# rasoolims/ImageTranslate

Hardware: AMD Instinct MI355X
Metric: train tokens/sec (whole node), 6L enc-dec d=512 seq128 b64, 1/2/4/8 GPU (higher is better)
Workload: dtype bf16; 1 GPU; 6L/6L enc-dec d=512 h=8 ff=2048 V=30000, src[64,128] tgt[64,128], synthetic random-token MT; global_batch=64, seq_len=128, parallelism=dp1, distinct_batches=8, directions=2

## Files before the change

imagetranslate_amd/_lib.py:

```python
import ctypes
import os
from ctypes import POINTER, Structure, c_char_p, c_float, c_int, c_int32, c_int64, c_uint64, c_void_p

_HERE = os.path.dirname(os.path.abspath(__file__))
LIB_PATH = os.environ.get("IMT_LIB") or os.path.join(_HERE, "libimt_hip.so")

IMT_F32, IMT_BF16 = 0, 1
IMT_NT, IMT_NN, IMT_TN = 0, 1, 2
IMT_AUX_NONE, IMT_AUX_GELU_FWD, IMT_AUX_DGELU, IMT_AUX_SPLITK_WS = 0, 1, 2, 3


class GemmArgs(Structure):
    _fields_ = [
        ("dtype", c_int32), ("layout", c_int32),
        ("M", c_int32), ("N", c_int32), ("K", c_int32),
        ("A", c_void_p), ("lda", c_int64),
        ("B", c_void_p), ("ldb", c_int64),
        ("C", c_void_p), ("ldc", c_int64),
        ("c_dtype", c_int32), ("accumulate", c_int32),
        ("bias", c_void_p),
        ("resid", c_void_p), ("ldr", c_int64),
        ("aux", c_void_p), ("ldaux", c_int64),
        ("aux_mode", c_int32), ("split_k", c_int32),
        ("alpha", c_float), ("dropout_p", c_float),
# ... 126 lines not shown
        ("x", c_void_p), ("ldx", c_int64),
        ("w", c_void_p), ("ldw", c_int64),
        ("bias", c_void_p), ("target", c_void_p),
        ("logprob", c_void_p), ("lse", c_void_p),
        ("seg_offsets", c_void_p), ("n_seg", c_int32), ("normalize", c_int32),
        ("seg_score", c_void_p),
        ("ws", c_void_p), ("ws_bytes", c_int64),
    ]


_P = c_void_p
SIGNATURES = {
    "imt_version": (c_int, []),
    "imt_last_error": (c_char_p, []),
    "imt_gemm": (c_int, [POINTER(GemmArgs), _P]),
    "imt_gemm_grouped_tn": (c_int, [POINTER(GemmArgs), c_int, _P]),
    "imt_gemm_splitk_ws_bytes": (c_int64, []),
    "imt_gemm_bias_residual_ln_supported": (c_int, [c_int, c_int, c_int]),
    "imt_gemm_bias_residual_ln": (c_int, [c_int, _P, c_int64, _P, c_int64, _P, _P, c_int64, _P, _P, _P, _P, c_int64, _P, _P, c_int, c_int,
                                          c_int, c_float, c_float, c_uint64, _P]),
    "imt_colsum": (c_int, [c_int, _P, c_int64, c_int, c_int, _P, _P, _P]),
    "imt_layernorm_fwd": (c_int, [c_int, _P, _P, _P, _P, _P, _P, c_int, c_int, c_float, c_float, c_uint64, _P]),
    "imt_add_layernorm_fwd": (c_int, [c_int, _P, _P, _P, _P, _P, _P, _P, _P, c_int, c_int, c_float, c_float, c_uint64, _P]),
    "imt_embed_ln_fwd": (c_int, [c_int, _P, _P, _P, _P, _P, _P, _P, _P, _P, _P, _P, _P, c_int, c_int, c_int, c_int, c_int, c_int, c_float,
                                 c_float, c_uint64, _P]),
    "imt_layernorm_bwd": (c_int, [c_int, _P, _P, _P, _P, _P, _P, _P, _P, c_int, c_int, c_float, c_uint64, _P, c_float,
                                  c_uint64, _P, _P]),
    "imt_embed_fwd": (c_int, [c_int, _P, _P, _P, _P, _P, _P, _P, c_int, c_int, c_int, c_int, c_int, c_int, _P]),
    "imt_embed_bwd": (c_int, [c_int, _P, _P, _P, _P, _P, _P, _P, c_int, c_int, c_int, c_int64, _P]),
    "imt_attention_fwd": (c_int, [POINTER(AttnArgs), _P]),
    "imt_attention_bwd": (c_int, [POINTER(AttnArgs), _P]),
    "imt_attention_qkv_fwd_supported": (c_int, [c_int, c_int, c_int, c_int, c_int, c_int, c_int]),
    "imt_attention_qkv_fwd": (c_int, [POINTER(AttnArgs), _P, c_int64, _P, _P, c_int, _P]),
    "imt_gather_rows": (c_int, [c_int, _P, c_int64, _P, _P, c_int64, c_int, c_int, _P]),
    "imt_scatter_rows": (c_int, [c_int, _P, c_int64, _P, _P, c_int64, c_int, c_int, _P]),
    "imt_log_softmax_fwd": (c_int, [c_int, _P, c_int64, _P, c_int64, _P, c_int, c_int, _P]),
    "imt_log_softmax_bwd": (c_int, [_P, c_int64, _P, c_int64, c_int, _P, c_int64, c_int, c_int, _P]),
    "imt_smoothed_nll_fwd": (c_int, [_P, c_int64, _P, _P, c_int, c_int, c_float, c_int64, _P]),
    "imt_smoothed_nll_bwd": (c_int, [_P, _P, _P, c_int64, c_int, c_int, c_float, c_int64, _P]),
    "imt_xent_fused_fwd_bwd": (c_int, [c_int, _P, c_int64, _P, _P, c_int, c_int, c_float, c_int64, c_float, _P]),
    "imt_score_ws_bytes": (c_int64, [c_int, c_int]),
    "imt_score_supported": (c_int, [c_int, c_int, c_int]),
    "imt_score_rows": (c_int, [POINTER(ScoreArgs), _P]),
    "imt_scaled_sum": (c_int, [_P, c_int, c_float, _P, _P]),
    "imt_sumsq": (c_int, [_P, c_int64, _P, _P, _P]),
    "imt_ln_partial_reduce": (c_int, [_P, c_int, c_int, _P, _P, _P, _P]),
    "imt_clip_adam": (c_int, [_P, _P, _P, _P, _P, c_int64, _P, c_float, c_float, c_float, c_float, c_float, c_float,
                              c_int64, c_int, _P]),
    "imt_clip_scale": (c_int, [_P, c_int64, _P, c_float, c_float, _P]),
    "imt_cast_f32_to_bf16": (c_int, [_P, _P, c_int64, _P]),
    "imt_gated_mix": (c_int, [c_int, _P, _P, _P, _P, c_int64, c_int, _P]),
    "imt_add_rows_dropout": (c_int, [c_int, _P, c_int, _P, _P, c_int64, c_int, c_int, c_float, c_uint64, _P]),
    "imt_obj_rows": (c_int, [c_int, c_int, _P, _P, _P, _P, _P, _P, _P, c_int64, c_int, c_int, _P, _P]),
    "imt_relu_dropout": (c_int, [c_int, _P, c_int64, c_int, c_float, c_uint64, _P]),
    "imt_relu_dropout_bwd": (c_int, [c_int, _P, _P, _P, c_int64, c_int, c_float, c_uint64, _P]),
    "imt_obj_fold_w": (c_int, [_P, _P, c_int, c_int, _P]),
    "imt_obj_embed_grad": (c_int, [c_int, _P, _P, c_int64, _P, c_int64, c_int, _P]),
    "imt_gated_mix_bwd": (c_int, [c_int, _P, _P, _P, _P, _P, _P, _P, _P, c_int64, c_int, _P]),
    "imt_attn_pool_plan": (c_int, [c_int, c_int, c_int]),
    "imt_attn_pool_fwd": (c_int, [c_int, _P, _P, _P, _P, _P, _P, _P, c_int64, c_int, c_int, _P]),
    "imt_attn_pool_bwd": (c_int, [c_int, _P, _P, _P, _P, _P, _P, _P, _P, _P, _P, _P, _P, c_int64, c_int, c_int, _P]),
    "imt_contrastive": (c_int, [_P, _P, _P, _P, _P, _P, c_int, c_int, c_int, _P]),
    "imt_sent_pool_fwd": (c_int, [c_int, _P, _P, _P, _P, _P, _P, c_int64, c_int, c_int, c_float, c_uint64, _P]),
    "imt_sent_pool_bwd": (c_int, [c_int, _P, _P, _P, _P, _P, _P, _P, _P, _P, c_int64, c_int, c_int, c_float, c_uint64, _P]),
    "imt_l2_dist": (c_int, [c_int, _P, _P, _P, _P, _P, c_int, c_int64, _P]),
    "imt_comm_unique_id_bytes": (c_int, []),
# ... 66 lines not shown
```

imagetranslate_amd/csrc/attention.hip:

```cpp
#include <stdlib.h>
#include "mma.hpp"

namespace {

struct AttnP {
  int B, H, Tq, Tk;
  const void* Q; int64_t ldq;
  const void* K; int64_t ldk;
  const void* V; int64_t ldv;
  void* O; int64_t ldo;
  float* lse;
  const uint8_t* key_mask;
  const uint8_t* query_mask;
  const uint8_t* mask3d;
  int causal;
  float scale;
  uint32_t drop_thresh; float inv_keep; uint64_t seed;
  const void* dO; int64_t lddo;
  void* dQ; int64_t lddq;
  void* dK; int64_t lddk;
  void* dV; int64_t lddv;
  unsigned long long* trace;
  float* delta;
};
// ... 455 lines not shown
        float pv = (i < p.Tq && j < p.Tk) ? __expf(v - lse_t[il]) : 0.f;
        float dpv = dp[mt][e], pdv = pv;
        if (p.drop_thresh) {
          const bool keep = attn_drop_keep(attn_drop_word(dropout_key(p.seed), attn_pair_row(p, b, h, i) + (uint64_t)(j >> 1)), j, p.drop_thresh);
          dpv = keep ? dpv * p.inv_keep : 0.f;
          pdv = keep ? pv * p.inv_keep : 0.f;
        }
        pd[mt][e] = pdv;
        s[mt][e] = pv * (dpv - delta_t[il]);
      }
#pragma unroll
    for (int u = 0; u < AccOperand<T>::NFR; ++u) {
      const frag_t pf = AccOperand<T>::get(pd, u);
      const frag_t dsf = AccOperand<T>::get(s, u);
#pragma unroll
      for (int dt = 0; dt < NDT; ++dt) {
        mma16(dv[dt], AccOperand<T>::template lds<RB>(dOt, u, 16 * dt), pf);
        mma16(dk[dt], AccOperand<T>::template lds<RB>(Qt, u, 16 * dt), dsf);
      }
    }
    }
  }
  if (j < p.Tk) {
    T* dKb = reinterpret_cast<T*>(p.dK) + ((int64_t)b * p.Tk + j) * p.lddk + h * DH;
    T* dVb = reinterpret_cast<T*>(p.dV) + ((int64_t)b * p.Tk + j) * p.lddv + h * DH;
#pragma unroll
    for (int dt = 0; dt < NDT; ++dt) {
      Vec4<T>::store(dKb + 16 * dt + 4 * g, dk[dt] * p.scale);
      Vec4<T>::store(dVb + 16 * dt + 4 * g, dv[dt]);
    }
  }
}

template <int DH, bool MASK3D>
__global__ __launch_bounds__(512, 4) void attn_bwd_fused_kernel(AttnP p) {
  typedef bf16_t T;
  constexpr int RB = DH * 2, NS = RB / 64, NDT = DH / 16;
  typedef typename Frag<T>::type frag_t;
  extern __shared__ __attribute__((aligned(16))) char smem[];
  char* Qs = smem;
  char* dOs = Qs + 128 * RB;
  char* dST = dOs + 128 * RB;
  float* lse_s = reinterpret_cast<float*>(dST + 128 * 256);
  float* delta_s = lse_s + 128;
  uint8_t* qmask_s = reinterpret_cast<uint8_t*>(delta_s + 128);

  const int lid = imt_xcd_block(blockIdx.x, gridDim.x);
  const int b = lid / p.H, h = lid % p.H;
  const int wave = threadIdx.x >> 6, lane = threadIdx.x & 63, r = lane & 15, g = lane >> 4;
  const T* Qb = reinterpret_cast<const T*>(p.Q) + (int64_t)b * p.Tq * p.ldq + h * DH;
  const T* Kb = reinterpret_cast<const T*>(p.K) + (int64_t)b * p.Tk * p.ldk + h * DH;
  const T* Vb = reinterpret_cast<const T*>(p.V) + (int64_t)b * p.Tk * p.ldv + h * DH;
  const T* dOb = reinterpret_cast<const T*>(p.dO) + (int64_t)b * p.Tq * p.lddo + h * DH;
  const T* Ob = reinterpret_cast<const T*>(p.O) + (int64_t)b * p.Tq * p.ldo + h * DH;

  IMT_STAMP(p.trace, 0);
  const int k0 = 16 * wave;
  const int j = k0 + r;
  frag_t kf[NS], vf[NS];
  bool key_ok;
  {
    constexpr int CPR = RB / 16, NIT = 128 * CPR / 512;
    u32x4 vq[NIT], vo[NIT];
#pragma unroll
    for (int it = 0; it < NIT; ++it) {
      const int q = threadIdx.x + it * 512, tr = min(q / CPR, p.Tq - 1), c = q % CPR;
      vq[it] = *reinterpret_cast<const u32x4*>(Qb + (int64_t)tr * p.ldq + c * 8);
      vo[it] = *reinterpret_cast<const u32x4*>(dOb + (int64_t)tr * p.lddo + c * 8);
    }
    const int i = 16 * wave + r;
    frag_t of[NS], dof[NS];
    load_row_frags<T, DH>(of, Ob, p.ldo, 16 * wave, p.Tq);
    load_row_frags<T, DH>(dof, dOb, p.lddo, 16 * wave, p.Tq);
    load_row_frags<T, DH>(kf, Kb, p.ldk, k0, p.Tk);
    load_row_frags<T, DH>(vf, Vb, p.ldv, k0, p.Tk);
    const float lse_v = p.lse[((int64_t)b * p.H + h) * p.Tq + min(i, p.Tq - 1)];
    const uint8_t* qmp = p.query_mask ? p.query_mask + (int64_t)b * p.Tq + min(i, p.Tq - 1) : reinterpret_cast<const uint8_t*>(Qb);
    const uint8_t* kmp = p.key_mask ? p.key_mask + (int64_t)b * p.Tk + min(j, p.Tk - 1) : reinterpret_cast<const uint8_t*>(Kb);
    const uint8_t qmv = *qmp, kmv = *kmp;
#pragma unroll
    for (int it = 0; it < NIT; ++it) {
      const int q = threadIdx.x + it * 512, tr = q / CPR, c = q % CPR;
      const u32x4 z = {0u, 0u, 0u, 0u};
      *reinterpret_cast<u32x4*>(Qs + tile_off<RB>(tr, c)) = (tr < p.Tq) ? vq[it] : z;
      *reinterpret_cast<u32x4*>(dOs + tile_off<RB>(tr, c)) = (tr < p.Tq) ? vo[it] : z;
    }
    float d = 0.f;
#pragma unroll
    for (int ks = 0; ks < NS; ++ks)
#pragma unroll
      for (int e = 0; e < 8; ++e) d += (float)dof[ks][e] * (float)of[ks][e];
    d += __shfl_xor(d, 16, 64);
    d += __shfl_xor(d, 32, 64);
    if (g == 0) {
      delta_s[i] = d;
      lse_s[i] = lse_v;
      qmask_s[i] = (i < p.Tq && p.query_mask) ? qmv : (uint8_t)1;
    }
    key_ok = (j < p.Tk) ? (p.key_mask ? (kmv != 0) : true) : false;
  }
  __syncthreads();
  IMT_STAMP(p.trace, 1);

  f32x4 dk[NDT], dv[NDT];
#pragma unroll
  for (int dt = 0; dt < NDT; ++dt) { dk[dt] = f32x4{0.f, 0.f, 0.f, 0.f}; dv[dt] = f32x4{0.f, 0.f, 0.f, 0.f}; }
  const int nqt = (p.Tq + 63) / 64;
#pragma unroll 1
  for (int qt = 0; qt < 2; ++qt) {
    const char* Qt = Qs + qt * 64 * RB;
    const char* dOt = dOs + qt * 64 * RB;
    f32x4 s[4], dp[4], pd[4];
    if (qt < nqt) {
#pragma unroll
      for (int mt = 0; mt < 4; ++mt) {
        s[mt] = f32x4{0.f, 0.f, 0.f, 0.f};
        dp[mt] = f32x4{0.f, 0.f, 0.f, 0.f};
#pragma unroll
// ... 50 lines not shown
    T* dKb = reinterpret_cast<T*>(p.dK) + ((int64_t)b * p.Tk + j) * p.lddk + h * DH;
    T* dVb = reinterpret_cast<T*>(p.dV) + ((int64_t)b * p.Tk + j) * p.lddv + h * DH;
#pragma unroll
    for (int dt = 0; dt < NDT; ++dt) {
      Vec4<T>::store(dKb + 16 * dt + 4 * g, dk[dt] * p.scale);
      Vec4<T>::store(dVb + 16 * dt + 4 * g, dv[dt]);
    }
  }
  IMT_STAMP(p.trace, 2);
  __syncthreads();
  IMT_STAMP(p.trace, 3);
  char* Ks = Qs;
#pragma unroll
  for (int ks = 0; ks < NS; ++ks) *reinterpret_cast<frag_t*>(Ks + tile_off<RB>(k0 + r, 4 * ks + g)) = kf[ks];
  __syncthreads();

  f32x4 dq[NDT];
#pragma unroll
  for (int dt = 0; dt < NDT; ++dt) dq[dt] = f32x4{0.f, 0.f, 0.f, 0.f};
  const int nks = (p.Tk + 31) / 32;
#pragma unroll 1
  for (int kstep = 0; kstep < nks; ++kstep) {
    const frag_t fa = lds_frag_kstrided_bf16<256>(dST, 32 * kstep, 16 * wave);
#pragma unroll
    for (int dt = 0; dt < NDT; ++dt) mma16(dq[dt], lds_frag_kstrided_bf16<RB>(Ks, 32 * kstep, 16 * dt), fa);
  }
  const int i = 16 * wave + r;
  if (i < p.Tq) {
    T* dQb = reinterpret_cast<T*>(p.dQ) + ((int64_t)b * p.Tq + i) * p.lddq + h * DH;
#pragma unroll
    for (int dt = 0; dt < NDT; ++dt) Vec4<T>::store(dQb + 16 * dt + 4 * g, dq[dt] * p.scale);
  }  IMT_STAMP(p.trace, 4);
}

template <int DH, bool MASK3D>
__global__ __launch_bounds__(512, 2) void attn_bwd_fused256_kernel(AttnP p) {
  typedef bf16_t T;
  constexpr int RB = DH * 2, NS = RB / 64, NDT = DH / 16, CPR = RB / 16;
  typedef typename Frag<T>::type frag_t;
  extern __shared__ __attribute__((aligned(16))) char smem[];
  char* Ks = smem;
  char* Qt = Ks + 256 * RB;
  char* dOt = Qt + 64 * RB;
  char* dST = dOt + 64 * RB;
  float* lse_s = reinterpret_cast<float*>(dST + 256 * 128);
  float* delta_s = lse_s + 256;
  uint8_t* qmask_s = reinterpret_cast<uint8_t*>(delta_s + 256);

  const int lid = imt_xcd_block(blockIdx.x, gridDim.x);
  const int b = lid / p.H, h = lid % p.H;
  const int wave = threadIdx.x >> 6, lane = threadIdx.x & 63, r = lane & 15, g = lane >> 4;
  const T* Qb = reinterpret_cast<const T*>(p.Q) + (int64_t)b * p.Tq * p.ldq + h * DH;
  const T* Kb = reinterpret_cast<const T*>(p.K) + (int64_t)b * p.Tk * p.ldk + h * DH;
  const T* Vb = reinterpret_cast<const T*>(p.V) + (int64_t)b * p.Tk * p.ldv + h * DH;
  const T* dOb = reinterpret_cast<const T*>(p.dO) + (int64_t)b * p.Tq * p.lddo + h * DH;
  const T* Ob = reinterpret_cast<const T*>(p.O) + (int64_t)b * p.Tq * p.ldo + h * DH;
  const int nqt = (p.Tq + 63) / 64;

  frag_t kf[2][NS], vf[2][NS];
  bool key_ok[2];
  const int st_row = (int)threadIdx.x / CPR, st_c = (int)threadIdx.x % CPR;
  const bool stager = st_row < 64;
  u32x4 vq, vo;
  auto prefetch = [&](int qt) {
    const int tr = min(qt * 64 + min(st_row, 63), p.Tq - 1);
    vq = *reinterpret_cast<const u32x4*>(Qb + (int64_t)tr * p.ldq + st_c * 8);
// ... 318 lines not shown
    if (p.drop_thresh) {
      const uint32_t key = dropout_key(p.seed);
      const uint32_t prow = (uint32_t)attn_pair_row(p, b, h, i) + (uint32_t)(2 * gq);
#pragma unroll
      for (int nt8 = 0; nt8 < 8; ++nt8)
#pragma unroll
        for (int e2 = 0; e2 < 2; ++e2) {
          const uint32_t w = attn_drop_word(key, prow + 8 * nt8 + e2);
          s[nt8][2 * e2] = (w & 0xffffu) >= p.drop_thresh ? s[nt8][2 * e2] * p.inv_keep : 0.f;
          s[nt8][2 * e2 + 1] = (w >> 16) >= p.drop_thresh ? s[nt8][2 * e2 + 1] * p.inv_keep : 0.f;
        }
    }
    psum += __shfl_xor(psum, 16, 64);
    psum += __shfl_xor(psum, 32, 64);
    f32x4 o[NDT];
#pragma unroll
    for (int dt = 0; dt < NDT; ++dt) o[dt] = f32x4{0.f, 0.f, 0.f, 0.f};
#pragma unroll
    for (int u = 0; u < 4; ++u) {
      const frag_t pf = acc_pair_to_frag(s[2 * u], s[2 * u + 1]);
#pragma unroll
      for (int dt = 0; dt < NDT; ++dt) mma16(o[dt], lds_frag_kperm_bf16<RB>(Vs, 32 * u, 16 * dt), pf);
    }
    const float inv_l = 1.0f / psum;
    if (i < p.Tq) {
      T* Ob = reinterpret_cast<T*>(p.O) + ((int64_t)b * p.Tq + i) * p.ldo + h * DH;
#pragma unroll
      for (int dt = 0; dt < NDT; ++dt) Vec4<T>::store(Ob + 16 * dt + 4 * gq, o[dt] * inv_l);
      if (gq == 0 && p.lse) p.lse[((int64_t)b * p.H + h) * p.Tq + i] = tmax + __logf(psum);
    }
  }
}

int check_args(const imt_attn_args* a, bool bwd) {
  IMT_CHECK_ARG(a != nullptr, "attention: null args");
  IMT_CHECK_ARG(imt_ok_dtype(a->dtype), "attention: bad dtype");
  IMT_CHECK_ARG(a->head_dim == 32 || a->head_dim == 64, "attention: head_dim %d unsupported (32 or 64)", a->head_dim);
  IMT_CHECK_ARG(a->B > 0 && a->H > 0 && a->Tq > 0 && a->Tk > 0, "attention: bad dims");
  const int al = (a->dtype == IMT_BF16) ? 8 : 4;
  IMT_CHECK_ARG(a->Q && a->K && a->V && a->O, "attention: null tensor");
  IMT_CHECK_ARG(a->ldq % al == 0 && a->ldk % al == 0 && a->ldv % al == 0 && a->ldo % al == 0, "attention: ld must be 16-B multiples");
  IMT_CHECK_ARG((((uintptr_t)a->Q | (uintptr_t)a->K | (uintptr_t)a->V | (uintptr_t)a->O) & 15) == 0, "attention: 16-B alignment");
  if (bwd) {
    IMT_CHECK_ARG(a->dO && a->dQ && a->dK && a->dV && a->lse && a->delta, "attention_bwd: null tensor");
    IMT_CHECK_ARG(a->lddo % al == 0 && a->lddq % al == 0 && a->lddk % al == 0 && a->lddv % al == 0, "attention_bwd: ld alignment");
    IMT_CHECK_ARG((((uintptr_t)a->dO | (uintptr_t)a->dQ | (uintptr_t)a->dK | (uintptr_t)a->dV) & 15) == 0, "attention_bwd: 16-B alignment");
  }
  return IMT_OK;
}

AttnP make_params(const imt_attn_args* a) {
  AttnP p;
  p.B = a->B; p.H = a->H; p.Tq = a->Tq; p.Tk = a->Tk;
  p.Q = a->Q; p.ldq = a->ldq; p.K = a->K; p.ldk = a->ldk; p.V = a->V; p.ldv = a->ldv; p.O = a->O; p.ldo = a->ldo;
  p.lse = a->lse; p.key_mask = a->key_mask; p.query_mask = a->query_mask; p.mask3d = a->mask3d; p.causal = a->causal;
  p.scale = a->scale;
  p.drop_thresh = dropout_thresh(a->dropout_p);
  p.inv_keep = a->dropout_p > 0.f ? 1.f / (1.f - a->dropout_p) : 1.f;
  p.seed = a->dropout_seed;
  p.dO = a->dO; p.lddo = a->lddo; p.dQ = a->dQ; p.lddq = a->lddq; p.dK = a->dK; p.lddk = a->lddk; p.dV = a->dV; p.lddv = a->lddv; p.trace = nullptr;
  p.delta = a->delta;
  return p;
}

template <typename T, int DH> int fwd_launch(const AttnP& p, hipStream_t st) {
  dim3 grid(imt_cdiv(p.Tq, 64) * p.H * p.B);
  const double work = (double)p.B * p.H * p.Tq * p.Tk * DH;
  const double io = ((double)p.B * p.H * DH * sizeof(T)) * (2.0 * p.Tq + 2.0 * p.Tk);
  ImtProfScope prof(sizeof(T) == 2 ? "attn_fwd_bf16" : "attn_fwd_f32", 4.0 * work, io, st);
  if (p.mask3d) hipLaunchKernelGGL((attn_fwd_kernel<T, DH, true>), grid, dim3(256), 0, st, p);
  else          hipLaunchKernelGGL((attn_fwd_kernel<T, DH, false>), grid, dim3(256), 0, st, p);
  IMT_CHECK_LAUNCH();
  return IMT_OK;
}
template <int DH, bool MASK3D> int bwd_fused_launch(const AttnP& p, hipStream_t st) {
  const double work = (double)p.B * p.H * p.Tq * p.Tk * DH;
  const double io = ((double)p.B * p.H * DH * 2.0) * (4.0 * p.Tq + 4.0 * p.Tk);
// ... 59 lines not shown
    AttnP pt = p;
    pt.trace = tr.dev;
    if (a->head_dim == 32) {
      if (p.mask3d) hipLaunchKernelGGL((attn_fwd_short_kernel<32, true>), dim3(p.B * p.H), dim3(512), 0, st, pt);
      else          hipLaunchKernelGGL((attn_fwd_short_kernel<32, false>), dim3(p.B * p.H), dim3(512), 0, st, pt);
    } else {
      if (p.mask3d) hipLaunchKernelGGL((attn_fwd_short_kernel<64, true>), dim3(p.B * p.H), dim3(512), 0, st, pt);
      else          hipLaunchKernelGGL((attn_fwd_short_kernel<64, false>), dim3(p.B * p.H), dim3(512), 0, st, pt);
    }
    IMT_CHECK_LAUNCH();
    return IMT_OK;
  }
  return a->head_dim == 32 ? fwd_launch<bf16_t, 32>(p, st) : fwd_launch<bf16_t, 64>(p, st);
}

extern "C" int imt_attention_bwd(const imt_attn_args* a, void* stream) {
  int rc = check_args(a, true);
  if (rc) return rc;
  const AttnP p = make_params(a);
  hipStream_t st = (hipStream_t)stream;
  if (a->dtype == IMT_F32) return a->head_dim == 32 ? bwd_launch<float, 32>(p, st) : bwd_launch<float, 64>(p, st);
  const bool idx32 = (double)a->B * a->H * a->Tq * a->Tk < 4294967296.0;
  if (a->Tq <= 128 && a->Tk <= 128 && idx32 && !getenv("IMT_ATTN_NO_FUSED_BWD")) {
    if (p.mask3d) return a->head_dim == 32 ? bwd_fused_launch<32, true>(p, st) : bwd_fused_launch<64, true>(p, st);
    return a->head_dim == 32 ? bwd_fused_launch<32, false>(p, st) : bwd_fused_launch<64, false>(p, st);
  }
  if (a->Tq <= 256 && a->Tk <= 256 && idx32 && !getenv("IMT_ATTN_NO_FUSED_BWD") && !getenv("IMT_ATTN_NO_FUSED256")) {
    if (p.mask3d) return a->head_dim == 32 ? bwd_fused256_launch<32, true>(p, st) : bwd_fused256_launch<64, true>(p, st);
    return a->head_dim == 32 ? bwd_fused256_launch<32, false>(p, st) : bwd_fused256_launch<64, false>(p, st);
  }
  return a->head_dim == 32 ? bwd_launch<bf16_t, 32>(p, st) : bwd_launch<bf16_t, 64>(p, st);
}

extern "C" int imt_attention_qkv_fwd_supported(int dtype, int head_dim, int H, int Tq, int Tk, int d_model, int has_mask3d) {
  return dtype == IMT_BF16 && head_dim == 64 && H % 2 == 0 && H * head_dim == d_model && Tq == Tk && Tq > 64 && Tq <= 128 &&
         d_model % 64 == 0 && d_model >= 128 && !has_mask3d;
}
extern "C" int imt_attention_qkv_fwd(const imt_attn_args* a, const void* x, int64_t ldx, const void* w, const void* bias, int d_model,
                                     void* stream) {
  int rc = check_args(a, false);
  if (rc) return rc;
  IMT_CHECK_ARG(x && w && ldx % 8 == 0 && (((uintptr_t)x | (uintptr_t)w) & 15) == 0, "attention_qkv_fwd: x / w missing or misaligned");
  IMT_CHECK_ARG(imt_attention_qkv_fwd_supported(a->dtype, a->head_dim, a->H, a->Tq, a->Tk, d_model, a->mask3d != nullptr),
                "attention_qkv_fwd: unsupported shape (bf16, head_dim 64, even heads, 64 < T <= 128, self-attention, no 3-D mask)");
  IMT_CHECK_ARG((double)a->B * a->H * a->Tq * a->Tk < 4294967296.0 && (int64_t)a->B * a->Tq * ldx * 2 < (1ll << 31) &&
                (int64_t)3 * d_model * d_model * 2 < (1ll << 31), "attention_qkv_fwd: operand too large for 32-bit offsets");
  const AttnP p = make_params(a);
  QkvP g;
  g.x = x; g.ldx = ldx; g.x_bytes = ((int64_t)(a->B * a->Tq - 1) * ldx + d_model) * 2; g.w = w; g.bias = bias; g.d_model = d_model;
  hipStream_t st = (hipStream_t)stream;
  const int lds = 2 * 65536;
  static bool attr_set = false;
  if (!attr_set) {
    (void)hipFuncSetAttribute(reinterpret_cast<const void*>(attn_qkv_fwd_kernel<false>), hipFuncAttributeMaxDynamicSharedMemorySize, lds);
    attr_set = true;
  }
  const double work = (double)p.B * p.H * p.Tq * p.Tk * a->head_dim;
  ImtProfScope prof("attn_qkv_fwd_bf16", 4.0 * work + 2.0 * p.B * p.Tq * 3.0 * d_model * d_model,
                    ((double)p.B * p.Tq * d_model * 2.0) * 5.0 + 6.0 * d_model * d_model, st);
  hipLaunchKernelGGL((attn_qkv_fwd_kernel<false>), dim3(p.B * (p.H / 2)), dim3(512), lds, st, p, g);
  IMT_CHECK_LAUNCH();
  return IMT_OK;
}
```

imagetranslate_amd/csrc/model.hip:

```cpp
#include "common.hpp"
#include "decode_fused.hpp"

namespace {

struct Carver {
  char* base; int64_t off;
  explicit Carver(void* b) : base(reinterpret_cast<char*>(b)), off(0) {}
  void* take(int64_t bytes) {
    void* p = base ? base + off : nullptr;
    off += (bytes + 255) & ~(int64_t)255;
    return p;
  }
};

struct AttnWs {
  void* qkv;
  void* kv;
  int64_t kv_ld;
  void* ctx;
  float* lse;
  void* pre_ln;
  float* mean; float* rstd;
  void* out;
};
// ... 223 lines not shown
    attn_args(c, a, B, T, T, w.qkv, 3 * d, offp(w.qkv, d, c.es), 3 * d, offp(w.qkv, 2 * d, c.es), 3 * d, w.ctx, w.lse, ms, ap,
              site_seed(seed, layer, site0));
    static const bool qkv_fusion = getenv("IMT_ATTN_QKV_FUSION") && atoi(getenv("IMT_ATTN_QKV_FUSION")) != 0;
    if (qkv_fusion && p.qkv_b >= 0 && imt_attention_qkv_fwd_supported(c.dtype, a.head_dim, a.H, T, T, d, ms.m3d != nullptr) &&
        (int64_t)B * T * d * c.es < (1ll << 31)) {
      RC(imt_attention_qkv_fwd(&a, x, d, c.P(p.qkv_w), c.P(p.qkv_b), d, c.st));
      RC(dense_resid_ln(c, w.ctx, d, N, d, p.o_w, p.o_b, d, x, p.ln_g, p.ln_b, w.pre_ln, w.out, w.mean, w.rstd, hp, site_seed(seed, layer, site0 + 1)));
      return IMT_OK;
    }
    RC(linear_fwd(c, x, d, N, d, p.qkv_w, p.qkv_b, 3 * d, w.qkv, 3 * d, nullptr, 0, nullptr, IMT_AUX_NONE, 0.f, 0));
  } else {
    const int Nk = B * Tk;
    RC(linear_fwd(c, x, d, N, d, p.qkv_w, p.qkv_b, d, w.qkv, d, nullptr, 0, nullptr, IMT_AUX_NONE, 0.f, 0));
    if (!kv_ready)
      RC(linear_fwd(c, kv_src, d, Nk, d, kv_w, kv_b, 2 * d, w.kv, w.kv_ld, nullptr, 0, nullptr, IMT_AUX_NONE, 0.f, 0));
    attn_args(c, a, B, T, Tk, w.qkv, d, w.kv, w.kv_ld, offp(w.kv, d, c.es), w.kv_ld, w.ctx, w.lse, ms, ap, site_seed(seed, layer, site0));
  }
  RC(imt_attention_fwd(&a, c.st));
  RC(dense_resid_ln(c, w.ctx, d, N, d, p.o_w, p.o_b, d, x, p.ln_g, p.ln_b, w.pre_ln, w.out, w.mean, w.rstd, hp, site_seed(seed, layer, site0 + 1)));
  return IMT_OK;
}

int attn_block_bwd(const Ctx& c, const imt_attn_block& p, AttnWs& w, StackWs& sw, DeferredDW& dw, int slot, const void* x, int B, int T,
                   const void* kv_src, int Tk, const MaskSet& ms, bool training, uint64_t seed, int layer, int site0, const void* dy,
                   void* d_kv_src, int accumulate_kv, int64_t kv_w = -1, int64_t kv_b = -1, void* d_kv_batched = nullptr) {
  const int d = c.m->d;
  const int N = B * T;
  const float hp = training ? c.m->hidden_dropout : 0.f, ap = training ? c.m->attn_dropout : 0.f;
  void* d_pre = sw.dpre[slot];
  void* d_dense = (hp > 0.f) ? sw.ddrop[slot] : d_pre;
  RC(imt_layernorm_bwd(c.dtype, dy, w.pre_ln, c.P(p.ln_g), w.mean, w.rstd, d_pre, c.G(p.ln_g), c.G(p.ln_b), N, d, 0.f, 0,
                       (hp > 0.f) ? d_dense : nullptr, hp, site_seed(seed, layer, site0 + 1), sw.ln_site(3 * layer + slot, d), c.st));
  dw.add(c, d_dense, d, w.ctx, d, N, d, d, p.o_w, p.o_b);
  RC(linear_bwd_input(c, d_dense, d, N, d, p.o_w, d, sw.d_ctx, d, nullptr, 0, nullptr, IMT_AUX_NONE, 0));
  imt_attn_args a;
  if (!kv_src) {
    attn_args(c, a, B, T, T, w.qkv, 3 * d, offp(w.qkv, d, c.es), 3 * d, offp(w.qkv, 2 * d, c.es), 3 * d, w.ctx, w.lse, ms, ap,
              site_seed(seed, layer, site0));
    a.dO = sw.d_ctx; a.lddo = d;
    a.dQ = sw.d_qkv; a.lddq = 3 * d; a.dK = offp(sw.d_qkv, d, c.es); a.lddk = 3 * d; a.dV = offp(sw.d_qkv, 2 * d, c.es); a.lddv = 3 * d;
    a.delta = sw.delta;
    RC(imt_attention_bwd(&a, c.st));
    dw.add(c, sw.d_qkv, 3 * d, x, d, N, 3 * d, d, p.qkv_w, p.qkv_b);
    RC(linear_bwd_input(c, sw.d_qkv, 3 * d, N, 3 * d, p.qkv_w, d, sw.d_run, d, d_pre, d, nullptr, IMT_AUX_NONE, 0));
  } else {
    const int Nk = B * Tk;
    attn_args(c, a, B, T, Tk, w.qkv, d, w.kv, w.kv_ld, offp(w.kv, d, c.es), w.kv_ld, w.ctx, w.lse, ms, ap, site_seed(seed, layer, site0));
    a.dO = sw.d_ctx; a.lddo = d;
    void* dkv = d_kv_batched ? d_kv_batched : sw.d_kv;
    const int64_t lddkv = d_kv_batched ? w.kv_ld : 2 * d;
    a.dQ = sw.d_q; a.lddq = d; a.dK = dkv; a.lddk = lddkv; a.dV = offp(dkv, d, c.es); a.lddv = lddkv;
    a.delta = sw.delta;
    RC(imt_attention_bwd(&a, c.st));
    dw.add(c, sw.d_q, d, x, d, N, d, d, p.qkv_w, p.qkv_b);
    RC(linear_bwd_input(c, sw.d_q, d, N, d, p.qkv_w, d, sw.d_run, d, d_pre, d, nullptr, IMT_AUX_NONE, 0));
    dw.add(c, dkv, lddkv, kv_src, d, Nk, 2 * d, d, kv_w, kv_b);
    if (!d_kv_batched) {
      if (d_kv_src)
        RC(linear_bwd_input(c, sw.d_kv, 2 * d, Nk, 2 * d, kv_w, d, d_kv_src, d, nullptr, 0, nullptr, IMT_AUX_NONE, accumulate_kv));
    }
  }
  return IMT_OK;
}

int ffn_fwd(const Ctx& c, const imt_layer_desc& p, LayerWs& w, const void* x, int N, bool training, uint64_t seed, int layer) {
  const int d = c.m->d, ff = c.m->ff;
  const float hp = training ? c.m->hidden_dropout : 0.f;
  RC(linear_fwd(c, x, d, N, d, p.ff1_w, p.ff1_b, ff, w.h, ff, nullptr, 0, w.z, IMT_AUX_GELU_FWD, 0.f, 0));
  RC(dense_resid_ln(c, w.h, ff, N, ff, p.ff2_w, p.ff2_b, d, x, p.ln2_g, p.ln2_b, w.pre_ln2, w.out, w.mean2, w.rstd2, hp, site_seed(seed, layer, 8)));
  return IMT_OK;
}

int ffn_bwd(const Ctx& c, const imt_layer_desc& p, LayerWs& w, StackWs& sw, DeferredDW& dw, const void* x, int N, bool training,
            uint64_t seed, int layer, const void* dy) {
  const int d = c.m->d, ff = c.m->ff;
  const float hp = training ? c.m->hidden_dropout : 0.f;
  void* d_pre = sw.dpre[0];
  void* d_dense = (hp > 0.f) ? sw.ddrop[0] : d_pre;
  RC(imt_layernorm_bwd(c.dtype, dy, w.pre_ln2, c.P(p.ln2_g), w.mean2, w.rstd2, d_pre, c.G(p.ln2_g), c.G(p.ln2_b), N, d, 0.f, 0,
                       (hp > 0.f) ? d_dense : nullptr, hp, site_seed(seed, layer, 8), sw.ln_site(3 * layer, d), c.st));
  dw.add(c, d_dense, d, w.h, ff, N, d, ff, p.ff2_w, p.ff2_b);
  RC(linear_bwd_input(c, d_dense, d, N, d, p.ff2_w, ff, sw.d_ff, ff, nullptr, 0, w.z, IMT_AUX_DGELU, 0));
  dw.add(c, sw.d_ff, ff, x, d, N, ff, d, p.ff1_w, p.ff1_b);
  RC(linear_bwd_input(c, sw.d_ff, ff, N, ff, p.ff1_w, d, sw.d_run, d, d_pre, d, nullptr, IMT_AUX_NONE, 0));
  return IMT_OK;
}
// ... 340 lines not shown
```

imagetranslate_amd/hip_ops.py:

```python
import ctypes
import os
import math

import torch

from . import _lib as L
from ._lib import IMT_AUX_DGELU, IMT_AUX_GELU_FWD, IMT_AUX_NONE, IMT_AUX_SPLITK_WS, IMT_BF16, IMT_F32, IMT_NN, IMT_NT, IMT_TN


def dt(t: torch.Tensor) -> int:
    if t.dtype == torch.float32:
        return IMT_F32
    if t.dtype == torch.bfloat16:
        return IMT_BF16
    raise TypeError("imagetranslate_amd supports float32 and bfloat16 tensors, got %s" % t.dtype)


def _stream():
    return ctypes.c_void_p(torch.cuda.current_stream().cuda_stream)


def _p(t):
    return None if t is None else ctypes.c_void_p(t.data_ptr())

# ... 225 lines not shown
def attention_qkv_fwd(x, w_qkv, b_qkv, B, H, T, head_dim, key_mask=None, query_mask=None, causal=False, scale=None,
                      dropout_p=0.0, dropout_seed=0):
    _req_cuda(x, w_qkv, b_qkv, key_mask, query_mask)
    d = H * head_dim
    qkv = torch.empty((B * T, 3 * d), device=x.device, dtype=x.dtype)
    a = _attn_args(qkv[:, :d], qkv[:, d:2 * d], qkv[:, 2 * d:], B, H, T, T, head_dim, key_mask, query_mask, None, causal, scale,
                   dropout_p, dropout_seed)
    o = torch.empty((B * T, d), device=x.device, dtype=x.dtype)
    lse = torch.empty((B, H, T), device=x.device, dtype=torch.float32)
    a.O, a.ldo, a.lse = o.data_ptr(), _rowmajor(o), lse.data_ptr()
    L.check(L.load().imt_attention_qkv_fwd(ctypes.byref(a), _p(x), _rowmajor(x), _p(w_qkv), _p(b_qkv), d, _stream()),
            "imt_attention_qkv_fwd")
    return qkv, o, lse


def attention_bwd(do, q, k, v, o, lse, B, H, Tq, Tk, head_dim, key_mask=None, query_mask=None, mask3d=None,
                  causal=False, scale=None, dropout_p=0.0, dropout_seed=0, dq=None, dk=None, dv=None):
    _req_cuda(do, q, k, v, o, lse)
    a = _attn_args(q, k, v, B, H, Tq, Tk, head_dim, key_mask, query_mask, mask3d, causal, scale, dropout_p, dropout_seed)
    if dq is None:
        dq = torch.empty((B * Tq, H * head_dim), device=q.device, dtype=q.dtype)
    if dk is None:
        dk = torch.empty((B * Tk, H * head_dim), device=q.device, dtype=q.dtype)
    if dv is None:
        dv = torch.empty((B * Tk, H * head_dim), device=q.device, dtype=q.dtype)
    delta = torch.empty((B, H, Tq), device=q.device, dtype=torch.float32)
    a.O, a.ldo, a.lse = o.data_ptr(), _rowmajor(o), lse.data_ptr()
    a.dO, a.lddo = do.data_ptr(), _rowmajor(do)
    a.dQ, a.lddq = dq.data_ptr(), _rowmajor(dq)
    a.dK, a.lddk = dk.data_ptr(), _rowmajor(dk)
    a.dV, a.lddv = dv.data_ptr(), _rowmajor(dv)
    a.delta = delta.data_ptr()
    L.check(L.load().imt_attention_bwd(ctypes.byref(a), _stream()), "imt_attention_bwd")
    return dq, dk, dv


def gather_rows(x, idx):
    _req_cuda(x, idx)
    out = torch.empty((idx.numel(), x.shape[1]), device=x.device, dtype=x.dtype)
    L.check(L.load().imt_gather_rows(dt(x), _p(x), _rowmajor(x), _p(idx), _p(out), out.stride(0) if out.numel() else x.shape[1],
                                     idx.numel(), x.shape[1], _stream()), "imt_gather_rows")
    return out


def scatter_rows(dout, idx, dx):
    _req_cuda(dout, idx, dx)
    L.check(L.load().imt_scatter_rows(dt(dout), _p(dout), _rowmajor(dout) if dout.numel() else dx.shape[1], _p(idx), _p(dx),
                                      _rowmajor(dx), idx.numel(), dx.shape[1], _stream()), "imt_scatter_rows")
    return dx


def log_softmax_fwd(logits):
    _req_cuda(logits)
    N, V = logits.shape
    lp = alloc_rows(N, V, torch.float32, logits.device)
    lse = torch.empty(N, device=logits.device, dtype=torch.float32)
    L.check(L.load().imt_log_softmax_fwd(dt(logits), _p(logits), _rowmajor(logits) if N else V, _p(lp), lp.stride(0) if N else V, _p(lse), N, V,
                                         _stream()), "imt_log_softmax_fwd")
    return lp, lse


_SCORE_WS = {}
SCORE_CHUNK_ROWS = 2048


def score_workspace(device, nbytes):
# ... 373 lines not shown
```

include/imt_hip.h:

```cpp
#ifndef IMT_HIP_H
#define IMT_HIP_H
#include <stdint.h>
#ifdef __cplusplus
extern "C" {
#endif

#define IMT_OK 0
#define IMT_ERR_BAD_ARG (-1)
#define IMT_ERR_UNSUPPORTED (-2)
#define IMT_ERR_LAUNCH (-3)

#define IMT_F32 0
#define IMT_BF16 1

int imt_version(void);
const char* imt_last_error(void);

int imt_abi_sizeof(const char* struct_name);

typedef struct imt_prof_row {
  char kind[48];
  int64_t launches;
  double total_ms;
  double flops;
// ... 73 lines not shown
                  const void* dsum, float* dword, float* dpos, float* dtype_tab, int n_tokens, int seq_len, int d,
                  int64_t pad_id, void* stream);
int imt_embed_ln_fwd(int dtype, const int64_t* ids, const int64_t* pos_ids, const int64_t* type_ids, const void* word,
                     const void* pos, const void* type, const void* gamma, const void* beta, void* sum_out, void* y,
                     float* mean, float* rstd, int n_tokens, int seq_len, int d, int vocab, int max_pos, int n_types, float eps,
                     float dropout_p, uint64_t dropout_seed, void* stream);

typedef struct imt_attn_args {
  int32_t dtype;
  int32_t B, H, Tq, Tk, head_dim;
  const void* Q; int64_t ldq;
  const void* K; int64_t ldk;
  const void* V; int64_t ldv;
  void* O; int64_t ldo;
  float* lse;
  const uint8_t* key_mask;
  const uint8_t* query_mask;
  const uint8_t* mask3d;
  int32_t causal;
  float scale;
  float dropout_p;
  uint64_t dropout_seed;
  const void* dO; int64_t lddo;
  void* dQ; int64_t lddq;
  void* dK; int64_t lddk;
  void* dV; int64_t lddv;
  float* delta;
} imt_attn_args;
int imt_attention_fwd(const imt_attn_args* a, void* stream);
int imt_attention_bwd(const imt_attn_args* a, void* stream);
int imt_attention_qkv_fwd_supported(int dtype, int head_dim, int H, int Tq, int Tk, int d_model, int has_mask3d);
int imt_attention_qkv_fwd(const imt_attn_args* a, const void* x, int64_t ldx, const void* w, const void* bias, int d_model,
                          void* stream);

int imt_gather_rows(int dtype, const void* x, int64_t ldx, const int32_t* idx, void* out, int64_t ldo, int n_sel,
                    int d, void* stream);
int imt_scatter_rows(int dtype, const void* dout, int64_t ldo, const int32_t* idx, void* dx, int64_t ldx, int n_sel,
                     int d, void* stream);

int imt_log_softmax_fwd(int dtype, const void* logits, int64_t ld, float* lp, int64_t ldlp, float* lse, int N, int V,
                        void* stream);
int imt_log_softmax_bwd(const float* dlp, int64_t lddlp, const float* lp, int64_t ldlp, int out_dtype, void* dlogits,
                        int64_t ld, int N, int V, void* stream);
int imt_smoothed_nll_fwd(const float* lp, int64_t ldlp, const int64_t* target, float* loss, int N, int V,
                         float epsilon, int64_t ignore_index, void* stream);
int imt_smoothed_nll_bwd(const float* dloss, const int64_t* target, float* dlp, int64_t lddlp, int N, int V,
                         float epsilon, int64_t ignore_index, void* stream);
int imt_xent_fused_fwd_bwd(int dtype, void* logits, int64_t ld, const int64_t* target, float* loss_rows, int N,
                           int V, float epsilon, int64_t ignore_index, float grad_scale, void* stream);

typedef struct imt_score_args {
  int32_t dtype;
  int32_t N, V, K;
  const void* x; int64_t ldx;
  const void* w; int64_t ldw;
  const void* bias;
  const int64_t* target;
  float* logprob;
  float* lse;
  const int64_t* seg_offsets;
  int32_t n_seg, normalize;
  float* seg_score;
  void* ws; int64_t ws_bytes;
} imt_score_args;
int64_t imt_score_ws_bytes(int N, int V);
int imt_score_supported(int dtype, int V, int K);
// ... 205 lines not shown
```

Baseline: 1.126 million tokens/s.

## Fuse output-projection input gradient into fused attention backward kernel

Adds an attention backward variant that computes each head's dO slice (dY times the head's W_o columns) inside the kernel, staging W_o chunks through shared memory with double buffering. This replaces the separate linear_bwd_input GEMM for the output projection and its round trip of d_ctx through global memory. The cost is that every head block rereads the full dY row and its W_o slice, which is redundant GEMM work spread across B*H blocks and may use more registers. It is on by default for bf16, head_dim 64, sequences up to 128 and no 3-D mask.

Measured after the change: 1.142 million tokens/s, median of 6. +1.4%, better.

```diff
diff --git a/imagetranslate_amd/_lib.py b/imagetranslate_amd/_lib.py
--- a/imagetranslate_amd/_lib.py
+++ b/imagetranslate_amd/_lib.py
@@ -182,6 +182,8 @@
     "imt_attention_bwd": (c_int, [POINTER(AttnArgs), _P]),
     "imt_attention_qkv_fwd_supported": (c_int, [c_int, c_int, c_int, c_int, c_int, c_int, c_int]),
     "imt_attention_qkv_fwd": (c_int, [POINTER(AttnArgs), _P, c_int64, _P, _P, c_int, _P]),
+    "imt_attention_bwd_proj_supported": (c_int, [c_int, c_int, c_int, c_int, c_int, c_int, c_int]),
+    "imt_attention_bwd_proj": (c_int, [POINTER(AttnArgs), _P, c_int64, _P, c_int64, c_int, _P]),
     "imt_gather_rows": (c_int, [c_int, _P, c_int64, _P, _P, c_int64, c_int, c_int, _P]),
     "imt_scatter_rows": (c_int, [c_int, _P, c_int64, _P, _P, c_int64, c_int, c_int, _P]),
     "imt_log_softmax_fwd": (c_int, [c_int, _P, c_int64, _P, c_int64, _P, c_int, c_int, _P]),
diff --git a/imagetranslate_amd/csrc/attention.hip b/imagetranslate_amd/csrc/attention.hip
--- a/imagetranslate_amd/csrc/attention.hip
+++ b/imagetranslate_amd/csrc/attention.hip
@@ -511,8 +511,10 @@
   }
 }
 
-template <int DH, bool MASK3D>
-__global__ __launch_bounds__(512, 4) void attn_bwd_fused_kernel(AttnP p) {
+struct ProjP { const void* dy; int64_t lddy; const void* w; int64_t ldw; int d_model; };
+
+template <int DH, bool MASK3D, bool PROJ>
+IMT_DEVICE void attn_bwd_fused_body(const AttnP& p, const ProjP& pj) {
   typedef bf16_t T;
   constexpr int RB = DH * 2, NS = RB / 64, NDT = DH / 16;
   typedef typename Frag<T>::type frag_t;
@@ -541,28 +543,95 @@
   {
     constexpr int CPR = RB / 16, NIT = 128 * CPR / 512;
     u32x4 vq[NIT], vo[NIT];
-#pragma unroll
-    for (int it = 0; it < NIT; ++it) {
-      const int q = threadIdx.x + it * 512, tr = min(q / CPR, p.Tq - 1), c = q % CPR;
-      vq[it] = *reinterpret_cast<const u32x4*>(Qb + (int64_t)tr * p.ldq + c * 8);
-      vo[it] = *reinterpret_cast<const u32x4*>(dOb + (int64_t)tr * p.lddo + c * 8);
-    }
     const int i = 16 * wave + r;
     frag_t of[NS], dof[NS];
-    load_row_frags<T, DH>(of, Ob, p.ldo, 16 * wave, p.Tq);
-    load_row_frags<T, DH>(dof, dOb, p.lddo, 16 * wave, p.Tq);
+    auto load_q_o = [&]() {
+#pragma unroll
+      for (int it = 0; it < NIT; ++it) {
+        const int q = threadIdx.x + it * 512, tr = min(q / CPR, p.Tq - 1), c = q % CPR;
+        vq[it] = *reinterpret_cast<const u32x4*>(Qb + (int64_t)tr * p.ldq + c * 8);
+        if (!PROJ) vo[it] = *reinterpret_cast<const u32x4*>(dOb + (int64_t)tr * p.lddo + c * 8);
+      }
+      load_row_frags<T, DH>(of, Ob, p.ldo, 16 * wave, p.Tq);
+    };
+    if (!PROJ) load_q_o();
+    if (!PROJ) load_row_frags<T, DH>(dof, dOb, p.lddo, 16 * wave, p.Tq);
     load_row_frags<T, DH>(kf, Kb, p.ldk, k0, p.Tk);
     load_row_frags<T, DH>(vf, Vb, p.ldv, k0, p.Tk);
     const float lse_v = p.lse[((int64_t)b * p.H + h) * p.Tq + min(i, p.Tq - 1)];
     const uint8_t* qmp = p.query_mask ? p.query_mask + (int64_t)b * p.Tq + min(i, p.Tq - 1) : reinterpret_cast<const uint8_t*>(Qb);
     const uint8_t* kmp = p.key_mask ? p.key_mask + (int64_t)b * p.Tk + min(j, p.Tk - 1) : reinterpret_cast<const uint8_t*>(Kb);
     const uint8_t qmv = *qmp, kmv = *kmp;
+    if constexpr (PROJ) {
+      static_assert(!PROJ || DH == 64, "the W_o slice is staged as 128-byte rows");
+      constexpr int WK = 256, WIT = WK * CPR / 512;
+      const int dm = pj.d_model, nks = dm / 32, nch = (nks + 7) / 8;
+      const T* Wb = reinterpret_cast<const T*>(pj.w) + h * DH + (threadIdx.x % CPR) * 8;
+      const T* dYr = reinterpret_cast<const T*>(pj.dy) + ((int64_t)b * p.Tq + min(i, p.Tq - 1)) * pj.lddy + 8 * g;
+      const int wkr = threadIdx.x / CPR;
+      u32x4 wv[WIT];
+      frag_t af[8];
+      auto load_w = [&](int ch) {
+#pragma unroll
+        for (int it = 0; it < WIT; ++it) wv[it] = *reinterpret_cast<const u32x4*>(Wb + (int64_t)min(WK * ch + wkr + 64 * it, dm - 1) * pj.ldw);
+      };
+      auto stage_w = [&](int ch) -> const char* {
+        char* Ws = (ch & 1) ? Qs : dST;
+#pragma unroll
+        for (int it = 0; it < WIT; ++it) *reinterpret_cast<u32x4*>(Ws + tile_off<RB>(wkr + 64 * it, threadIdx.x % CPR)) = wv[it];
+        __syncthreads();
+        return Ws;
+      };
+      load_w(0);
+#pragma unroll
+      for (int ks = 0; ks < 8; ++ks) af[ks] = *reinterpret_cast<const frag_t*>(dYr + min(32 * ks, dm - 32));
+      f32x4 acc[4];
+#pragma unroll
+      for (int nt = 0; nt < 4; ++nt) acc[nt] = f32x4{0.f, 0.f, 0.f, 0.f};
+#pragma unroll 1
+      for (int ch = 0; ch + 1 < nch; ++ch) {
+        const char* Ws = stage_w(ch);
+        load_w(ch + 1);
+#pragma unroll
+        for (int ks = 0; ks < 8; ++ks) {
+#pragma unroll
+          for (int nt = 0; nt < 4; ++nt) mma16(acc[nt], lds_frag_kstrided_bf16<RB>(Ws, 32 * ks, 16 * nt), af[ks]);
+          af[ks] = *reinterpret_cast<const frag_t*>(dYr + min(WK * (ch + 1) + 32 * ks, dm - 32));
+        }
+      }
+      {
+        const char* Ws = stage_w(nch - 1);
+        load_q_o();
+        const int nk = nks - 8 * (nch - 1);
+#pragma unroll
+        for (int ks = 0; ks < 8; ++ks) {
+          if (ks < nk) {
+#pragma unroll
+            for (int nt = 0; nt < 4; ++nt) mma16(acc[nt], lds_frag_kstrided_bf16<RB>(Ws, 32 * ks, 16 * nt), af[ks]);
+          }
+        }
+      }
+      __syncthreads();
+      T* dOg = (p.dO && i < p.Tq) ? const_cast<T*>(dOb) + (int64_t)i * p.lddo : nullptr;
+#pragma unroll
+      for (int nt = 0; nt < 4; ++nt) {
+        const f32x4 v = (i < p.Tq) ? acc[nt] : f32x4{0.f, 0.f, 0.f, 0.f};
+        const bf16x4 w = {(bf16_t)v[0], (bf16_t)v[1], (bf16_t)v[2], (bf16_t)v[3]};
+        const int col = 16 * nt + 4 * g;
+        *reinterpret_cast<bf16x4*>(dOs + tile_off<RB>(i, col >> 3) + ((col & 7) << 1)) = w;
+        if (dOg) *reinterpret_cast<bf16x4*>(dOg + col) = w;
+      }
+    }
 #pragma unroll
     for (int it = 0; it < NIT; ++it) {
       const int q = threadIdx.x + it * 512, tr = q / CPR, c = q % CPR;
       const u32x4 z = {0u, 0u, 0u, 0u};
       *reinterpret_cast<u32x4*>(Qs + tile_off<RB>(tr, c)) = (tr < p.Tq) ? vq[it] : z;
-      *reinterpret_cast<u32x4*>(dOs + tile_off<RB>(tr, c)) = (tr < p.Tq) ? vo[it] : z;
+      if (!PROJ) *reinterpret_cast<u32x4*>(dOs + tile_off<RB>(tr, c)) = (tr < p.Tq) ? vo[it] : z;
+    }
+    if constexpr (PROJ) {
+#pragma unroll
+      for (int s = 0; s < NS; ++s) dof[s] = lds_frag_kcontig<T, RB>(dOs, 16 * wave, 4 * s);
     }
     float d = 0.f;
 #pragma unroll
@@ -679,6 +748,14 @@
     for (int dt = 0; dt < NDT; ++dt) Vec4<T>::store(dQb + 16 * dt + 4 * g, dq[dt] * p.scale);
   }  IMT_STAMP(p.trace, 4);
 }
+template <int DH, bool MASK3D>
+__global__ __launch_bounds__(512, 4) void attn_bwd_fused_kernel(AttnP p) {
+  attn_bwd_fused_body<DH, MASK3D, false>(p, ProjP());
+}
+template <bool MASK3D>
+__global__ __launch_bounds__(512, 4) void attn_bwd_proj_kernel(AttnP p, ProjP pj) {
+  attn_bwd_fused_body<64, MASK3D, true>(p, pj);
+}
 
 template <int DH, bool MASK3D>
 __global__ __launch_bounds__(512, 2) void attn_bwd_fused256_kernel(AttnP p) {
@@ -1063,7 +1140,7 @@
   }
 }
 
-int check_args(const imt_attn_args* a, bool bwd) {
+int check_args(const imt_attn_args* a, bool bwd, bool need_dO = true) {
   IMT_CHECK_ARG(a != nullptr, "attention: null args");
   IMT_CHECK_ARG(imt_ok_dtype(a->dtype), "attention: bad dtype");
   IMT_CHECK_ARG(a->head_dim == 32 || a->head_dim == 64, "attention: head_dim %d unsupported (32 or 64)", a->head_dim);
@@ -1073,7 +1150,7 @@
   IMT_CHECK_ARG(a->ldq % al == 0 && a->ldk % al == 0 && a->ldv % al == 0 && a->ldo % al == 0, "attention: ld must be 16-B multiples");
   IMT_CHECK_ARG((((uintptr_t)a->Q | (uintptr_t)a->K | (uintptr_t)a->V | (uintptr_t)a->O) & 15) == 0, "attention: 16-B alignment");
   if (bwd) {
-    IMT_CHECK_ARG(a->dO && a->dQ && a->dK && a->dV && a->lse && a->delta, "attention_bwd: null tensor");
+    IMT_CHECK_ARG((a->dO || !need_dO) && a->dQ && a->dK && a->dV && a->lse && a->delta, "attention_bwd: null tensor");
     IMT_CHECK_ARG(a->lddo % al == 0 && a->lddq % al == 0 && a->lddk % al == 0 && a->lddv % al == 0, "attention_bwd: ld alignment");
     IMT_CHECK_ARG((((uintptr_t)a->dO | (uintptr_t)a->dQ | (uintptr_t)a->dK | (uintptr_t)a->dV) & 15) == 0, "attention_bwd: 16-B alignment");
   }
@@ -1199,6 +1276,41 @@
   return a->head_dim == 32 ? bwd_launch<bf16_t, 32>(p, st) : bwd_launch<bf16_t, 64>(p, st);
 }
 
+extern "C" int imt_attention_bwd_proj_supported(int dtype, int head_dim, int H, int Tq, int Tk, int d_model, int has_mask3d) {
+  const bool fused_off = getenv("IMT_ATTN_NO_FUSED_BWD") != nullptr;
+  return dtype == IMT_BF16 && head_dim == 64 && H > 0 && H * 64 == d_model && Tq > 0 && Tq <= 128 && Tk > 0 && Tk <= 128 &&
+         !has_mask3d && !fused_off;
+}
+extern "C" int imt_attention_bwd_proj(const imt_attn_args* a, const void* dy, int64_t lddy, const void* w_o, int64_t ldw, int d_model,
+                                      void* stream) {
+  int rc = check_args(a, true, false);
+  if (rc) return rc;
+  IMT_CHECK_ARG(imt_attention_bwd_proj_supported(a->dtype, a->head_dim, a->H, a->Tq, a->Tk, d_model, a->mask3d != nullptr),
+                "attention_bwd_proj: unsupported shape (bf16, head_dim 64, T <= 128, d_model = 64 H, no 3-D mask)");
+  IMT_CHECK_ARG(dy && w_o && lddy >= d_model && ldw >= d_model && lddy % 8 == 0 && ldw % 8 == 0 &&
+                (((uintptr_t)dy | (uintptr_t)w_o) & 15) == 0, "attention_bwd_proj: dy / w_o missing, misaligned or narrower than d_model");
+  IMT_CHECK_ARG((double)a->B * a->H * a->Tq * a->Tk < 4294967296.0, "attention_bwd_proj: too many score elements for 32-bit dropout indices");
+  const AttnP p = make_params(a);
+  ProjP pj;
+  pj.dy = dy; pj.lddy = lddy; pj.w = w_o; pj.ldw = ldw; pj.d_model = d_model;
+  hipStream_t st = (hipStream_t)stream;
+  const int lds = 2 * 128 * 64 * 2 + 128 * 256 + 128 * 4 * 2 + 128;
+  static bool attr_set = false;
+  if (!attr_set) {
+    (void)hipFuncSetAttribute(reinterpret_cast<const void*>(attn_bwd_proj_kernel<false>), hipFuncAttributeMaxDynamicSharedMemorySize, lds);
+    attr_set = true;
+  }
+  const double work = (double)p.B * p.H * p.Tq * p.Tk * 64.0;
+  ImtProfScope prof("attn_bwd_fused_bf16", 10.0 * work + 2.0 * p.B * p.Tq * (double)d_model * d_model,
+                    ((double)p.B * p.H * 64 * 2.0) * (3.0 * p.Tq + 4.0 * p.Tk) + 2.0 * p.B * p.Tq * d_model + 2.0 * d_model * d_model, st);
+  ImtTrace tr("attn_bwd", p.B * p.H, st);
+  AttnP pt = p;
+  pt.trace = tr.dev;
+  hipLaunchKernelGGL((attn_bwd_proj_kernel<false>), dim3(p.B * p.H), dim3(512), lds, st, pt, pj);
+  IMT_CHECK_LAUNCH();
+  return IMT_OK;
+}
+
 extern "C" int imt_attention_qkv_fwd_supported(int dtype, int head_dim, int H, int Tq, int Tk, int d_model, int has_mask3d) {
   return dtype == IMT_BF16 && head_dim == 64 && H % 2 == 0 && H * head_dim == d_model && Tq == Tk && Tq > 64 && Tq <= 128 &&
          d_model % 64 == 0 && d_model >= 128 && !has_mask3d;
diff --git a/imagetranslate_amd/csrc/model.hip b/imagetranslate_amd/csrc/model.hip
--- a/imagetranslate_amd/csrc/model.hip
+++ b/imagetranslate_amd/csrc/model.hip
@@ -279,7 +279,14 @@
   RC(imt_layernorm_bwd(c.dtype, dy, w.pre_ln, c.P(p.ln_g), w.mean, w.rstd, d_pre, c.G(p.ln_g), c.G(p.ln_b), N, d, 0.f, 0,
                        (hp > 0.f) ? d_dense : nullptr, hp, site_seed(seed, layer, site0 + 1), sw.ln_site(3 * layer + slot, d), c.st));
   dw.add(c, d_dense, d, w.ctx, d, N, d, d, p.o_w, p.o_b);
-  RC(linear_bwd_input(c, d_dense, d, N, d, p.o_w, d, sw.d_ctx, d, nullptr, 0, nullptr, IMT_AUX_NONE, 0));
+  static const bool do_fusion = !(getenv("IMT_ATTN_DO_FUSION") && atoi(getenv("IMT_ATTN_DO_FUSION")) == 0);
+  const bool proj = do_fusion && imt_attention_bwd_proj_supported(c.dtype, d / c.m->heads, c.m->heads, T, kv_src ? Tk : T, d, ms.m3d != nullptr);
+  if (!proj) RC(linear_bwd_input(c, d_dense, d, N, d, p.o_w, d, sw.d_ctx, d, nullptr, 0, nullptr, IMT_AUX_NONE, 0));
+  auto attn_bwd = [&](imt_attn_args& a) {
+    if (!proj) return imt_attention_bwd(&a, c.st);
+    a.dO = nullptr;
+    return imt_attention_bwd_proj(&a, d_dense, d, c.P(p.o_w), d, d, c.st);
+  };
   imt_attn_args a;
   if (!kv_src) {
     attn_args(c, a, B, T, T, w.qkv, 3 * d, offp(w.qkv, d, c.es), 3 * d, offp(w.qkv, 2 * d, c.es), 3 * d, w.ctx, w.lse, ms, ap,
@@ -287,7 +294,7 @@
     a.dO = sw.d_ctx; a.lddo = d;
     a.dQ = sw.d_qkv; a.lddq = 3 * d; a.dK = offp(sw.d_qkv, d, c.es); a.lddk = 3 * d; a.dV = offp(sw.d_qkv, 2 * d, c.es); a.lddv = 3 * d;
     a.delta = sw.delta;
-    RC(imt_attention_bwd(&a, c.st));
+    RC(attn_bwd(a));
     dw.add(c, sw.d_qkv, 3 * d, x, d, N, 3 * d, d, p.qkv_w, p.qkv_b);
     RC(linear_bwd_input(c, sw.d_qkv, 3 * d, N, 3 * d, p.qkv_w, d, sw.d_run, d, d_pre, d, nullptr, IMT_AUX_NONE, 0));
   } else {
@@ -298,7 +305,7 @@
     const int64_t lddkv = d_kv_batched ? w.kv_ld : 2 * d;
     a.dQ = sw.d_q; a.lddq = d; a.dK = dkv; a.lddk = lddkv; a.dV = offp(dkv, d, c.es); a.lddv = lddkv;
     a.delta = sw.delta;
-    RC(imt_attention_bwd(&a, c.st));
+    RC(attn_bwd(a));
     dw.add(c, sw.d_q, d, x, d, N, d, d, p.qkv_w, p.qkv_b);
     RC(linear_bwd_input(c, sw.d_q, d, N, d, p.qkv_w, d, sw.d_run, d, d_pre, d, nullptr, IMT_AUX_NONE, 0));
     dw.add(c, dkv, lddkv, kv_src, d, Nk, 2 * d, d, kv_w, kv_b);
diff --git a/imagetranslate_amd/hip_ops.py b/imagetranslate_amd/hip_ops.py
--- a/imagetranslate_amd/hip_ops.py
+++ b/imagetranslate_amd/hip_ops.py
@@ -281,6 +281,27 @@
     a.dV, a.lddv = dv.data_ptr(), _rowmajor(dv)
     a.delta = delta.data_ptr()
     L.check(L.load().imt_attention_bwd(ctypes.byref(a), _stream()), "imt_attention_bwd")
+    return dq, dk, dv
+
+
+def attention_bwd_proj(dy, w_o, q, k, v, o, lse, B, H, Tq, Tk, head_dim, key_mask=None, query_mask=None, causal=False,
+                       scale=None, dropout_p=0.0, dropout_seed=0, do_out=None):
+    _req_cuda(dy, w_o, q, k, v, o, lse, do_out)
+    d = H * head_dim
+    a = _attn_args(q, k, v, B, H, Tq, Tk, head_dim, key_mask, query_mask, None, causal, scale, dropout_p, dropout_seed)
+    dq = torch.empty((B * Tq, d), device=q.device, dtype=q.dtype)
+    dk = torch.empty((B * Tk, d), device=q.device, dtype=q.dtype)
+    dv = torch.empty((B * Tk, d), device=q.device, dtype=q.dtype)
+    delta = torch.empty((B, H, Tq), device=q.device, dtype=torch.float32)
+    a.O, a.ldo, a.lse = o.data_ptr(), _rowmajor(o), lse.data_ptr()
+    if do_out is not None:
+        a.dO, a.lddo = do_out.data_ptr(), _rowmajor(do_out)
+    a.dQ, a.lddq = dq.data_ptr(), _rowmajor(dq)
+    a.dK, a.lddk = dk.data_ptr(), _rowmajor(dk)
+    a.dV, a.lddv = dv.data_ptr(), _rowmajor(dv)
+    a.delta = delta.data_ptr()
+    L.check(L.load().imt_attention_bwd_proj(ctypes.byref(a), _p(dy), _rowmajor(dy), _p(w_o), _rowmajor(w_o), d, _stream()),
+            "imt_attention_bwd_proj")
     return dq, dk, dv
 
 
diff --git a/include/imt_hip.h b/include/imt_hip.h
--- a/include/imt_hip.h
+++ b/include/imt_hip.h
@@ -129,6 +129,9 @@
 int imt_attention_qkv_fwd_supported(int dtype, int head_dim, int H, int Tq, int Tk, int d_model, int has_mask3d);
 int imt_attention_qkv_fwd(const imt_attn_args* a, const void* x, int64_t ldx, const void* w, const void* bias, int d_model,
                           void* stream);
+int imt_attention_bwd_proj_supported(int dtype, int head_dim, int H, int Tq, int Tk, int d_model, int has_mask3d);
+int imt_attention_bwd_proj(const imt_attn_args* a, const void* dy, int64_t lddy, const void* w_o, int64_t ldw, int d_model,
+                           void* stream);
 
 int imt_gather_rows(int dtype, const void* x, int64_t ldx, const int32_t* idx, void* out, int64_t ldo, int n_sel,
                     int d, void* stream);
```
